# TencentCloudADP/youtu-rag

Hardware: AMD Instinct MI355X
Metric: retrieval QPS + recall@10 vs CPU ref, 10M×1024 corpus, 1/2/4/8 MI355X (higher is better)
Workload: dtype bf16

## Files before the change

youtu-rag_amd/csrc/hr_index.hip:

```cpp
#include "hr_internal.hpp"
#include "hr_kernels.hpp"

static thread_local std::string g_err;
int set_err(int code, const std::string& msg) {
    g_err = msg;
    return code;
}

static int async_drain(hr_index* h);

struct Persist {
    int mode = 1;
    bool ready = false;
    int64_t key_n = -1;
    const void* key_rows = nullptr;
    int key_S = 0, key_P = 0, key_ncu = 0;
    Scratch slot[kPersistSlots];
    DevBuf ar_qfrag, ar_mkeys, ar_floor, ar_pbuf, ar_pcnt, ar_dynq;
    int64_t st_qfrag = 0, st_mkeys = 0, st_floor = 0, st_pbuf = 0, st_pcnt = 0, st_dynq = 0;
    DevBuf ctl;
    uint32_t* host_err = nullptr;
    hipStream_t pst = nullptr;
    hipEvent_t posted[kPersistSlots] = {};
    hipEvent_t closed = nullptr;
// ... 429 lines not shown
    std::lock_guard<std::mutex> lk(h->mu);
    if (int rc = async_drain(h)) return rc;
    if (h->n + n > max_rows(h)) return set_err(HR_E_INVALID, "a shard holds at most 2^32 rows");
    if (n == 0) {
        if (first_row_out) *first_row_out = h->n;
        return HR_OK;
    }
    if (h->G > 1) return group_add_device(h, rows_dev, n, first_row_out, (hipStream_t)stream);
    if (int rc = set_device(h)) return rc;
    hipEvent_t ev;
    HIP_TRY(hipEventCreateWithFlags(&ev, hipEventDisableTiming));
    hipError_t e = hipEventRecord(ev, (hipStream_t)stream);
    if (e == hipSuccess) e = hipStreamWaitEvent(h->stream, ev, 0);
    (void)hipEventDestroy(ev);
    HIP_TRY(e);
    return add_impl<ADD_DEVICE>(h, rows_dev, 0, 0, n, first_row_out);
}

extern "C" int hr_index_remove(hr_index* h, const int64_t* rows, int64_t n) {
    if (!h || n < 0 || (n > 0 && !rows)) return set_err(HR_E_INVALID, "bad arguments");
    std::lock_guard<std::mutex> lk(h->mu);
    if (int rc = async_drain(h)) return rc;
    if (h->G > 1) return group_remove(h, rows, n);
    return index_remove_local(h, rows, n);
}

int index_remove_local(hr_index* h, const int64_t* rows, int64_t n) {
    if (int rc = set_device(h)) return rc;
    for (int64_t i = 0; i < n; ++i)
        if (rows[i] < 0 || rows[i] >= h->n) return set_err(HR_E_INVALID, "row out of range");
    int64_t lo = INT64_MAX, hi = -1;
    for (int64_t i = 0; i < n; ++i) {
        const int64_t r = rows[i];
        uint32_t& w = h->live_host[(size_t)(r >> 5)];
        const uint32_t bit = 1u << (r & 31);
        if (w & bit) {
            w &= ~bit;
            h->n_live--;
        }
        lo = std::min(lo, r >> 5);
        hi = std::max(hi, r >> 5);
    }
    if (hi >= 0) {
        HIP_TRY(hipMemcpyAsync(h->live + lo, h->live_host.data() + lo, (size_t)(hi - lo + 1) * 4,
                               hipMemcpyHostToDevice, h->stream));
        HIP_TRY(hipStreamSynchronize(h->stream));
    }
    return HR_OK;
}

extern "C" int hr_index_size(hr_index* h, int64_t* n_out, int64_t* n_live_out) {
    if (!h) return set_err(HR_E_INVALID, "null handle");
    std::lock_guard<std::mutex> lk(h->mu);
    if (n_out) *n_out = h->n;
    int64_t live = h->n_live;
    if (h->G > 1) {
        live = 0;
        for (hr_index* s : h->shards) live += s->n_live;
    }
    if (n_live_out) *n_live_out = live;
    return HR_OK;
}

extern "C" int hr_index_info(hr_index* h, int* dim_out, int* dtype_out, int* metric_out, int* n_dev_out) {
    if (!h) return set_err(HR_E_INVALID, "null handle");
    if (dim_out) *dim_out = h->dim;
    if (dtype_out) *dtype_out = h->dtype;
    if (metric_out) *metric_out = h->metric;
    if (n_dev_out) *n_dev_out = h->G;
    return HR_OK;
}

static int knob(const char* name, int dflt) {
    const char* v = getenv(name);
    return v && *v ? atoi(v) : dflt;
}
static const int kTailCus = knob("HIPRAG_TAIL_CUS", 32);
static const int kSampleMin = knob("HIPRAG_SAMPLE_MIN", 1024);
static const int kDynPct = knob("HIPRAG_DYN_PCT", 10);
static const int kRefreshEvery = std::max(0, knob("HIPRAG_REFRESH_EVERY", 0));
static int refresh_every(int64_t n_tiles) { return kRefreshEvery ? kRefreshEvery : (n_tiles <= 160 * 1024 ? 8 : 4); }
static const int kRefreshEvery8 = std::max(0, knob("HIPRAG_REFRESH_EVERY8", 0));
static int refresh_every8() { return kRefreshEvery8 ? kRefreshEvery8 : (kRefreshEvery ? kRefreshEvery : 16); }

struct Plan {
    int QB, Bp, P;
    int NG;
};

static int scan_lds_bytes(const hr_index* h, int QB) { return h->S * QB * 1024; }

static int make_plan(const hr_index* h, int B, Plan* p) {
    const int QB = (B > 32 && scan_lds_bytes(h, 2) <= 160 * 1024) ? 2 : 1;
    if (scan_lds_bytes(h, QB) > 160 * 1024)
        return set_err(HR_E_UNSUPPORTED, "dim too large for the LDS-resident query tile (max 2560)");
    p->QB = QB;
    constexpr int max_groups = 4;
    const int sdt = scan_dtype(h);
    p->NG = (QB == 2 && (sdt != F32 || wide_filter_ok(sdt, h->S))) ? std::max(1, std::min(max_groups, (B + 63) / 64)) : 1;
    if (QB == 1 && B > 32 && sdt != F32) p->NG = std::max(1, std::min(max_groups, (B + 31) / 32));
    if (p->NG > 1 && QB == 2 && wide_filter_ok(sdt, h->S)) p->NG = (p->NG + 1) & ~1;
    p->Bp = p->NG * QB * 32;
    const int pmax = sdt == F32 ? (QB == 2 ? 4 : 8) : 16;
    p->P = (h->S % 16 == 0 && pmax >= 16) ? 16 : (h->S % 8 == 0 && pmax >= 8 ? 8 : 4);
    return HR_OK;
}

static bool wide_plan(const hr_index* h, const Plan& pl, int np, bool tile_list) {
    const bool f32 = scan_dtype(h) == F32;
    const int max_parts = std::min(f32 ? 7 : 3, wide_max_parts(scan_dtype(h)));
    const bool parts_ok = np <= max_parts && (f32 || pl.NG == 2);
    return pl.NG >= 2 && pl.QB == 2 && !tile_list && (np == 1 || parts_ok) && wide_filter_ok(scan_dtype(h), h->S);
}

static void set_dyn_tail(ScanArgs& args, int64_t W, uint32_t* dyn_q) {
    const int pct = kDynPct;
    const int64_t per_wave = args.n_units / W;
    args.dyn_start = args.n_units;
    if (per_wave >= 8 && dyn_q) {
        const int64_t s_per = per_wave - std::max<int64_t>(2, per_wave * pct / 100);
        args.dyn_start = s_per * W;
        args.dyn_pct = pct;
        args.dyn_chunk = 2;
        args.dyn_q = dyn_q;
    }
}

template <int MT, int DT, int QB, int P, int MODE, bool NT, int TPB = kScanThreads, bool QM = false>
static int launch_scan_t(hr_index* h, Scratch& sc, int cus, const ScanArgs& a, hipStream_t st, int lds) {
    const int ng = std::max(1, a.ng);
    auto kern = scan_kernel<MT, DT, QB, P, MODE, NT, TPB, QM>();
    static std::mutex attr_mu;
    static int attr_lds[64] = {};
    static int occ[64][4] = {};
    const int dev = h->device & 63;
    const int bucket = lds <= 40 * 1024 ? 0 : lds <= 80 * 1024 ? 1 : lds <= 120 * 1024 ? 2 : 3;
    int per_cu;
    {
        std::lock_guard<std::mutex> lk(attr_mu);
        if (attr_lds[dev] < 160 * 1024) {
            HIP_TRY(hipFuncSetAttribute((const void*)kern, hipFuncAttributeMaxDynamicSharedMemorySize, 160 * 1024));
            attr_lds[dev] = 160 * 1024;
        }
        if (!occ[dev][bucket]) {
            int o = 0;
            HIP_TRY(hipOccupancyMaxActiveBlocksPerMultiprocessor(&o, kern, TPB, lds));
            occ[dev][bucket] = std::max(1, o);
        }
        per_cu = occ[dev][bucket];
    }
    int64_t blocks = std::max<int64_t>(1, std::min<int64_t>((int64_t)cus * per_cu / ng, (a.n_units + 7) / 8));
    if (ng > 1) blocks = std::max<int64_t>(8, blocks / 8 * 8);
    ScanArgs args = a;
    args.ng = ng;
    if (MODE == SCAN_FILTER) {
        const int64_t W = blocks * (TPB / 64);
        const int Bq = QB * 32;
        HIP_TRY(sc.pbuf.ensure((size_t)ng * Bq * W * kCapW * sizeof(float2)));
        HIP_TRY(sc.pcnt.ensure((size_t)ng * Bq * W * 4));
        HIP_TRY(sc.wtiles.ensure((size_t)ng * W * 4));
        args.wave_tiles = sc.wtiles.as<uint32_t>();
        sc.wtiles_valid = true;
        args.pbuf = sc.pbuf.as<float2>();
        args.pcnt = sc.pcnt.as<uint32_t>();
        args.capw = kCapW;
        sc.last_W = W;
        sc.last_Bp = Bq;
        sc.last_ng = ng;
        sc.last_capw = kCapW;
        h->last_scr = &sc;
        set_dyn_tail(args, W, sc.dyn_q.as<uint32_t>());
    }
    hipLaunchKernelGGL(kern, dim3((unsigned)(blocks * ng)), dim3(TPB), lds, st, args);
    HIP_TRY(hipGetLastError());
    return HR_OK;
}

template <int MT, int DT, int MODE>
static int launch_scan_p(hr_index* h, Scratch& sc, int cus, const Plan& pl, const ScanArgs& a, hipStream_t st,
                         bool qm = false) {
    int lds = scan_lds_bytes(h, pl.QB);
    if (MODE == SCAN_SAMPLE) lds = std::max(lds, (kScanThreads / 64) * pl.QB * 16 * 64 * 4 + 64);
    const bool dflt = pl.NG > 1 || MODE == SCAN_SAMPLE;
    if constexpr (MODE == SCAN_FILTER) {
        if (wide_plan(h, pl, a.np, a.tile_list != nullptr) && a.use_groups) {
            if (pl.NG == 4 && a.np == 1 && h->q256 && q256_filter_ok(scan_dtype(h), h->S)) {
                const int blocks = (int)std::max<int64_t>(1, std::min<int64_t>(cus, (a.n_units + 7) / 8));
                const int64_t W = (int64_t)blocks * 4;
                HIP_TRY(sc.pbuf.ensure((size_t)4 * 64 * W * kCapW * sizeof(float2)));
                HIP_TRY(sc.pcnt.ensure((size_t)4 * 64 * W * 4));
                sc.last_W = W;
                sc.last_Bp = 64;
                sc.last_ng = 4;
                sc.last_capw = kCapW;
                sc.wtiles_valid = false;
                h->last_scr = &sc;
                ScanArgs b = a;
                b.pbuf = sc.pbuf.as<float2>();
                b.pcnt = sc.pcnt.as<uint32_t>();
                b.capw = kCapW;
                if (int rc = launch_filter_q256(MT, DT, h->S, blocks, b, st)) return set_err(rc, "256-query FILTER launch failed");
                h->n_q256++;
                return HR_OK;
            }
            constexpr int wpb = 8;
            const int blocks = (int)std::max<int64_t>(1, std::min<int64_t>(cus, (a.n_units + wpb - 1) / wpb));
            const int64_t W = (int64_t)blocks * wpb;
            HIP_TRY(sc.pbuf.ensure((size_t)pl.NG * 64 * W * kCapW * sizeof(float2)));
            HIP_TRY(sc.pcnt.ensure((size_t)pl.NG * 64 * W * 4));
            sc.last_W = W;
            sc.last_Bp = 64;
            sc.last_ng = pl.NG;
            sc.last_capw = kCapW;
            sc.wtiles_valid = false;
            h->last_scr = &sc;
            for (int set = 0; set < pl.NG / 2; ++set) {
                ScanArgs b = a;
                b.qfrag = a.qfrag + (int64_t)set * 2 * h->S * 2 * 64 * 8;
                b.mkeys = a.mkeys + set * 128 * 32;
                b.floor_q = a.floor_q + set * 128;
                b.pbuf = sc.pbuf.as<float2>() + (int64_t)set * 2 * W * 64 * kCapW;
                b.pcnt = sc.pcnt.as<uint32_t>() + (int64_t)set * 2 * W * 64;
                b.capw = kCapW;
                if (int rc = launch_filter_wide(MT, DT, h->S, blocks, b, st)) return set_err(rc, "wide FILTER launch failed");
                h->n_wide++;
            }
            return HR_OK;
        }
    }
    if constexpr (MODE != SCAN_COLLECT) {
        if (qm) {
            if (pl.NG != 1 || !a.mask) return set_err(HR_E_INVALID, "per-query masks take one query group per pass");
            if (MODE == SCAN_FILTER) h->n_qmask++;
            constexpr bool QNT = MODE == SCAN_FILTER;
#define HR_SCAN_QM_CASE(QBv, Pv) \
    if (pl.QB == QBv && pl.P == Pv)  \
        return launch_scan_t<MT, DT, QBv, Pv, MODE, QNT, kScanThreads, true>(h, sc, cus, a, st, lds);
            if constexpr (DT == F32) {
                HR_SCAN_QM_CASE(1, 8) HR_SCAN_QM_CASE(1, 4) HR_SCAN_QM_CASE(2, 4)
            } else {
                HR_SCAN_QM_CASE(1, 16) HR_SCAN_QM_CASE(2, 16) HR_SCAN_QM_CASE(1, 8) HR_SCAN_QM_CASE(2, 8)
                HR_SCAN_QM_CASE(1, 4) HR_SCAN_QM_CASE(2, 4)
            }
#undef HR_SCAN_QM_CASE
            return set_err(HR_E_INVALID, "no per-query-mask scan variant for this plan");
        }
    }
#define HR_SCAN_CASE(QBv, Pv)                                                                     \
    if (pl.QB == QBv && pl.P == Pv)                                                               \
        return dflt ? launch_scan_t<MT, DT, QBv, Pv, MODE, false>(h, sc, cus, a, st, lds)         \
                    : launch_scan_t<MT, DT, QBv, Pv, MODE, true>(h, sc, cus, a, st, lds);
    if constexpr (DT == F32) {
        HR_SCAN_CASE(1, 8) HR_SCAN_CASE(1, 4) HR_SCAN_CASE(2, 4)
    } else {
        HR_SCAN_CASE(1, 16) HR_SCAN_CASE(2, 16) HR_SCAN_CASE(1, 8) HR_SCAN_CASE(2, 8) HR_SCAN_CASE(1, 4)
        HR_SCAN_CASE(2, 4)
    }
#undef HR_SCAN_CASE
    return set_err(HR_E_INVALID, "no scan variant for this plan");
}

static int launch_scan(hr_index* h, Scratch& sc, int cus, const Plan& pl, const ScanArgs& a, int mode,
                       hipStream_t st, bool qm = false) {
    return dispatch_dt(scan_dtype(h), [&](auto dt) -> int {
        constexpr int DT = decltype(dt)::value;
        auto go = [&](auto mt) -> int {
            constexpr int MT = decltype(mt)::value;
            if (mode == SCAN_SAMPLE) return launch_scan_p<MT, DT, SCAN_SAMPLE>(h, sc, cus, pl, a, st, qm);
            if (mode == SCAN_FILTER) return launch_scan_p<MT, DT, SCAN_FILTER>(h, sc, cus, pl, a, st, qm);
            return launch_scan_p<MT, DT, SCAN_COLLECT>(h, sc, cus, pl, a, st);
        };
        if constexpr (DT == F32) {
            if (mfma_type(h) == F16) return go(std::integral_constant<int, F16>{});
            return go(std::integral_constant<int, BF16>{});
        } else {
            return go(std::integral_constant<int, DT == F16 ? F16 : BF16>{});
        }
    });
}

template <int MODE>
static int launch_scan8(hr_index* h, Scratch& sc, int cus, const Plan& pl, const ScanArgs& a, hipStream_t st) {
    static_assert(MODE == SCAN_SAMPLE || MODE == SCAN_FILTER, "the collect pass reads the 16-bit rows");
    int lds = scan_lds_bytes(h, pl.QB);
    if (MODE == SCAN_SAMPLE) lds = std::max(lds, (kScanThreads / 64) * pl.QB * 16 * 64 * 4 + 64);
    const int S8 = h->S / 2;
    const int P8 = S8 % 16 == 0 ? 16 : (S8 % 8 == 0 ? 8 : (S8 % 4 == 0 ? 4 : 2));
    constexpr bool NT = MODE == SCAN_FILTER;
    if (MODE == SCAN_FILTER) h->n_shadow8++;
#define HR_SCAN8_CASE(QBv, Pv) \
    if (pl.QB == QBv && P8 == Pv) return launch_scan_t<F16, I8S, QBv, Pv, MODE, NT>(h, sc, cus, a, st, lds);
    HR_SCAN8_CASE(2, 16) HR_SCAN8_CASE(1, 16) HR_SCAN8_CASE(2, 8) HR_SCAN8_CASE(1, 8) HR_SCAN8_CASE(2, 4)
    HR_SCAN8_CASE(1, 4) HR_SCAN8_CASE(2, 2) HR_SCAN8_CASE(1, 2)
#undef HR_SCAN8_CASE
    return set_err(HR_E_INVALID, "no shadow-8 scan variant for this plan");
}

static int tail_cus(const hr_index* h) {
    return std::max(0, std::min(kTailCus, h->n_cu - 8));
}

static int persist_quiesce(hr_index* h) {
    Persist* ps = h->ps;
    if (!ps || !(ps->active || ps->launched)) return HR_OK;
    if (int rc = set_device(h)) return rc;
    PersistCtl* c = ps->ctl.as<PersistCtl>();
    if (ps->active)
        if (int rc = launch_persist_close(c, h->pre)) return rc;
    HIP_TRY(hipStreamSynchronize(h->pre));
    HIP_TRY(hipStreamSynchronize(ps->pst));
    HIP_TRY(hipMemsetAsync(&c->stop, 0, 4, ps->pst));
    HIP_TRY(hipStreamSynchronize(ps->pst));
    ps->active = ps->launched = false;
    if (ps->host_err && *(volatile uint32_t*)ps->host_err) {
        ps->timeouts++;
        ps->last_err = *(volatile uint32_t*)ps->host_err;
        *(volatile uint32_t*)ps->host_err = 0;
        HIP_TRY(hipMemset(&c->error, 0, 4));
    }
    return HR_OK;
}

static int persist_close(hr_index* h) {
    Persist* ps = h->ps;
    if (!ps || !ps->active) return HR_OK;
    if (int rc = set_device(h)) return rc;
    if (int rc = launch_persist_close(ps->ctl.as<PersistCtl>(), h->pre)) return rc;
    HIP_TRY(hipEventRecord(ps->closed, h->pre));
    HIP_TRY(hipStreamWaitEvent(ps->pst, ps->closed, 0));
    HIP_TRY(hipMemsetAsync(&ps->ctl.as<PersistCtl>()->stop, 0, 4, ps->pst));
    ps->active = false;
    return HR_OK;
}

static void persist_free(hr_index* h) {
    Persist* ps = h->ps;
    if (!ps) return;
    (void)persist_quiesce(h);
    ps->drop_views();
    for (auto& sc : ps->slot) sc.release_all();
    for (DevBuf* b : {&ps->ar_qfrag, &ps->ar_mkeys, &ps->ar_floor, &ps->ar_pbuf, &ps->ar_pcnt, &ps->ar_dynq, &ps->ctl})
        b->release();
    for (auto& e : ps->posted)
        if (e) (void)hipEventDestroy(e);
    if (ps->closed) (void)hipEventDestroy(ps->closed);
    if (ps->pst) (void)hipStreamDestroy(ps->pst);
    if (ps->host_err) (void)hipHostFree(ps->host_err);
    delete ps;
    h->ps = nullptr;
}

static bool persist_wanted(hr_index* h, const Plan& pl, int np, bool early, const uint64_t* mask_dev, int64_t n_tiles) {
    const int mode = h->ps ? h->ps->mode : 1;
    if (mode == 0 || !early || mask_dev || np != 1 || pl.NG != 1 || pl.QB != 2 || h->stripe_G != 1) return false;
    if (!(scan_dtype(h) != F32 ? pl.P == 16 : pl.P == 4)) return false;
    return mode == 2 || (n_tiles >= 128 * 1024 && n_tiles <= 160 * 1024);
}

static int persist_configure(hr_index* h, const Plan& pl) {
    if (!h->ps) h->ps = new Persist();
    Persist& ps = *h->ps;
    const int64_t n_tiles = (h->n + 31) / 32;
    const int nwg = h->n_cu - tail_cus(h);
    if (ps.ready && ps.key_n == h->n && ps.key_rows == h->rows && ps.key_S == h->S && ps.key_P == pl.P &&
        ps.key_ncu == h->n_cu)
        return HR_OK;
    if (int rc = persist_quiesce(h)) return rc;
    if ((n_tiles + 7) / 8 < nwg) return set_err(HR_E_UNSUPPORTED, "shard too small for the persistent FILTER");
    if (!ps.pst) {
        HIP_TRY(index_stream_create(h, &ps.pst, true));
        for (auto& e : ps.posted) HIP_TRY(hipEventCreateWithFlags(&e, hipEventDisableTiming));
        HIP_TRY(hipEventCreateWithFlags(&ps.closed, hipEventDisableTiming));
        HIP_TRY(hipHostMalloc((void**)&ps.host_err, 64));
        *ps.host_err = 0;
// ... 2073 lines not shown
```

youtu-rag_amd/csrc/hr_kernels.hpp:

```cpp
#pragma once
#include "hr_common.hpp"

namespace hr {

template <int DT, bool SYNTH>
__global__ __launch_bounds__(256) void k_store(const float* __restrict__ in, uint64_t seed, int64_t gen_base, int64_t n,
                                               int dim, int S, int metric, int64_t lrow0, uint8_t* __restrict__ rows,
                                               unsigned long long* max_norm2_bits,
                                               const int64_t* __restrict__ dest = nullptr, int sG = 1, int ss = 0) {
    const int lane = threadIdx.x & 63;
    const int64_t r = (int64_t)blockIdx.x * 4 + (threadIdx.x >> 6);
    if (r >= n) return;
    const int64_t grow = SYNTH ? gen_base + stripe_row(lrow0 + r, sG, ss) : 0;
    auto src = [&](int d) -> float {
        if (d >= dim) return 0.0f;
        return SYNTH ? gen_elem(seed, grow, dim, d) : in[r * dim + d];
    };
    double inv = 1.0;
    bool scale = false;
    if (metric == COSINE) {
        double p = 0.0;
        for (int d = lane; d < dim; d += 64) {
            double x = (double)src(d);
            p = p + x * x;
// ... 116 lines not shown
    }
    double e1 = 0.0, nh = 0.0, qn = 0.0;
    const int qg = (b >> 5) / QB, qb = (b >> 5) % QB;
    auto put = [&](int d, float x) {
        const float y = scale ? (float)((double)x * inv) : x;
        q32[(int64_t)b * dpad + d] = y;
        const uint16_t h = quant_mt<MT>(y);
        const float dq = dequant_mt<MT>(h);
        const int s = d >> 4, sl = (b & 31) + 32 * ((d >> 3) & 1), jj = d & 7;
        qfrag[((((int64_t)qg * S + s) * QB + qb) * 64 + sl) * 8 + jj] = h;
        const double e = (double)y - (double)dq;
        e1 += e * e;
        nh += (double)dq * (double)dq;
        qn = qn + (double)y * (double)y;
    };
#pragma unroll
    for (int j = 0; j < kPrepJ; ++j)
        if (lane + 64 * j < dpad) put(lane + 64 * j, v[j]);
    for (int d = lane + 64 * kPrepJ; d < dpad; d += 64) put(d, src(d));
    e1 = wave_butterfly_sum(e1);
    nh = wave_butterfly_sum(nh);
    qn = wave_butterfly_sum(qn);
    if (lane == 0) {
        qerr[4 * b] = __builtin_sqrt(e1);
        qerr[4 * b + 1] = __builtin_sqrt(nh);
        qerr[4 * b + 2] = qn;
        qerr[4 * b + 3] = 0.0;
    }
}

constexpr int vmcnt_only(int n) { return 0x0F70 | (n & 15) | (((n >> 4) & 3) << 14); }

__device__ inline void stage_lds(u32x4* dst, const u32x4* src, int n) {
    constexpr int U = 8;
    const int st = blockDim.x;
    int i = threadIdx.x;
    for (; i + (U - 1) * st < n; i += U * st) {
        u32x4 v[U];
#pragma unroll
        for (int j = 0; j < U; ++j) v[j] = src[i + j * st];
#pragma unroll
        for (int j = 0; j < U; ++j) dst[i + j * st] = v[j];
    }
    for (; i < n; i += st) dst[i] = src[i];
}

struct ScanArgs {
    const uint8_t* rows;
    const uint32_t* live;
    const uint32_t* mask;
    const uint16_t* qfrag;
    int S;
    int64_t n_units;
    int64_t sample_stride;
    const uint32_t* tile_list;
    uint32_t* mkeys;
    int np;
    int64_t part_tiles;
    int64_t pstride;
    const float* floor_q;
    int use_groups;
    uint32_t* cnt;
    float2* buf;
    int cap;
    int refresh_every;
    int publish;
    int private_bufs;
    int wave_major;
    int strided;
    float2* pbuf;
    uint32_t* pcnt;
    int capw;
    int64_t dyn_start;
    int dyn_chunk;
    uint32_t* dyn_q;
    const float* xnorm;
    uint32_t* wave_tiles;
    int ng;
    int early_refresh;
    int teams;
    int dyn_pct;
    int stagger;
    const float* rscale;
};


constexpr int kPersistSlots = 3;
constexpr int kPersistRing = 4096;
struct PersistCtl {
    uint32_t gate;
    uint32_t posted;
    uint32_t next_epoch;
    uint32_t stop;
    uint32_t error;
    uint32_t runs;
    uint32_t opened;
    uint32_t pad;
    uint32_t slot_fail[4];
    unsigned long long arr[kPersistRing];
    unsigned long long t_end[kPersistRing];
    unsigned long long t_post[kPersistRing], t_start0[kPersistRing], t_start1[kPersistRing], t_end0[kPersistRing];
};
struct PersistLaunch {
    ScanArgs a;
    int64_t st_qfrag, st_mkeys, st_floor, st_pbuf, st_pcnt, st_dynq;
    PersistCtl* ctl;
    uint32_t* host_err;
    uint32_t e0;
    uint32_t idle_ticks;
};

template <int MT>
__device__ inline f32x16 mfma32(const u32x4& a, const u32x4& b, const f32x16& c) {
    if constexpr (MT == BF16)
        return __builtin_amdgcn_mfma_f32_32x32x16_bf16(__builtin_bit_cast(bf16x8, a), __builtin_bit_cast(bf16x8, b), c,
                                                        0, 0, 0);
    else
        return __builtin_amdgcn_mfma_f32_32x32x16_f16(__builtin_bit_cast(f16x8, a), __builtin_bit_cast(f16x8, b), c, 0,
                                                       0, 0);
}

template <int MT, int DT, bool NT = true>
struct XFrag;
#ifndef HR_CORPUS_NT
#define HR_CORPUS_NT 1
#endif
#ifndef HR_DIAG
#define HR_DIAG 0
#endif
#ifndef HR_ROTATE_ROUNDS
#define HR_ROTATE_ROUNDS 1
#endif
__device__ inline int64_t wave_uniform(int64_t v) {
    const uint32_t lo = (uint32_t)__builtin_amdgcn_readfirstlane((int)(uint32_t)v);
    const uint32_t hi = (uint32_t)__builtin_amdgcn_readfirstlane((int)(uint32_t)((uint64_t)v >> 32));
    return (int64_t)(((uint64_t)hi << 32) | lo);
}
__device__ inline uint32_t scalar_word(const uint32_t* p, int64_t i) {
    return ((const __attribute__((address_space(4))) uint32_t*)p)[i];
}
template <bool NT>
__device__ inline u32x4 corpus_load(const uint8_t* p) {
#if HR_CORPUS_NT
    if constexpr (NT) return __builtin_nontemporal_load((const u32x4*)p);
#endif
    return *(const u32x4*)p;
}
template <int MT, bool NT>
struct XFrag<MT, BF16, NT> {
    static constexpr int kLoads = 1;
    static constexpr int kSteps = 1;
    u32x4 v;
    __device__ inline void load(const uint8_t* rows, int64_t c, int lane) {
        v = corpus_load<NT>(rows + c * 1024 + lane * 16);
    }
    __device__ inline u32x4 get(int = 0) const { return v; }
};
template <int MT, bool NT>
struct XFrag<MT, F16, NT> {
    static constexpr int kLoads = 1;
    static constexpr int kSteps = 1;
    u32x4 v;
    __device__ inline void load(const uint8_t* rows, int64_t c, int lane) {
        v = corpus_load<NT>(rows + c * 1024 + lane * 16);
    }
    __device__ inline u32x4 get(int = 0) const { return v; }
};
template <int MT, bool NT>
struct XFrag<MT, F32, NT> {
    static constexpr int kLoads = 2;
    static constexpr int kSteps = 1;
    u32x4 a, b;
    __device__ inline void load(const uint8_t* rows, int64_t c, int lane) {
        a = corpus_load<NT>(rows + c * 2048 + lane * 16);
        b = corpus_load<NT>(rows + c * 2048 + 1024 + lane * 16);
    }
    __device__ inline u32x4 get(int = 0) const {
        typedef float f32x4 __attribute__((ext_vector_type(4)));
        typedef float f32x8 __attribute__((ext_vector_type(8)));
        const f32x4 fa = __builtin_bit_cast(f32x4, a);
        const f32x4 fb = __builtin_bit_cast(f32x4, b);
        const f32x8 f = __builtin_shufflevector(fa, fb, 0, 1, 2, 3, 4, 5, 6, 7);
        if constexpr (MT == BF16) {
            return __builtin_bit_cast(u32x4, __builtin_convertvector(f, bf16x8));
        } else {
            return __builtin_bit_cast(u32x4, __builtin_convertvector(f, f16x8));
        }
    }
};

template <bool NT>
struct XFrag<F16, I8S, NT> {
    static constexpr int kLoads = 1;
    static constexpr int kSteps = 2;
    u32x4 v;
    __device__ inline void load(const uint8_t* rows, int64_t c, int lane) {
        v = corpus_load<NT>(rows + c * 1024 + lane * 16);
    }
    __device__ inline u32x4 get(int ks) const {
        typedef _Float16 f16x2 __attribute__((ext_vector_type(2)));
        const uint32_t w0 = ks ? v[2] : v[0], w1 = ks ? v[3] : v[1];
        const f16x2 off = {(_Float16)1152.0f, (_Float16)1152.0f};
        auto cv = [&](uint32_t w, uint32_t sel) -> uint32_t {
            const uint32_t m = __builtin_amdgcn_perm(0x64646464u, w, sel);
            return __builtin_bit_cast(uint32_t, __builtin_bit_cast(f16x2, m) - off);
        };
        u32x4 o;
        o[0] = cv(w0, 0x04010400u);
        o[1] = cv(w0, 0x04030402u);
        o[2] = cv(w1, 0x04010400u);
        o[3] = cv(w1, 0x04030402u);
        return o;
    }
};

__device__ inline int acc_query(int qb, int i, int half) { return qb * 32 + (i & 3) + 8 * (i >> 2) + 4 * half; }

template <int CTRL>
__device__ __forceinline__ uint32_t dpp_u32(uint32_t v) {
    return (uint32_t)__builtin_amdgcn_update_dpp((int)v, (int)v, CTRL, 0xF, 0xF, false);
}
__device__ __forceinline__ float half_min32(float f) {
    f = fminf(f, __builtin_bit_cast(float, dpp_u32<0xB1>(__builtin_bit_cast(uint32_t, f))));
    f = fminf(f, __builtin_bit_cast(float, dpp_u32<0x4E>(__builtin_bit_cast(uint32_t, f))));
    f = fminf(f, __builtin_bit_cast(float, dpp_u32<0x141>(__builtin_bit_cast(uint32_t, f))));
    f = fminf(f, __builtin_bit_cast(float, dpp_u32<0x140>(__builtin_bit_cast(uint32_t, f))));
    return fminf(f, __builtin_bit_cast(float, __builtin_amdgcn_ds_swizzle(__builtin_bit_cast(int, f), 0x401F)));
}
__device__ __forceinline__ uint32_t wave_or(uint32_t x) {
    x |= dpp_u32<0xB1>(x);
    x |= dpp_u32<0x4E>(x);
    x |= dpp_u32<0x141>(x);
    x |= dpp_u32<0x140>(x);
    return (uint32_t)(__builtin_amdgcn_readlane((int)x, 0) | __builtin_amdgcn_readlane((int)x, 16) |
                      __builtin_amdgcn_readlane((int)x, 32) | __builtin_amdgcn_readlane((int)x, 48));
}
__device__ __forceinline__ float half_kth_largest(float f, int j) {
    const int lane = __lane_id();
    for (int r = 0; r < 32 - j; ++r) {
        const float m = half_min32(f);
        const uint64_t b = __ballot(f == m);
        const uint32_t bh = lane >= 32 ? (uint32_t)(b >> 32) : (uint32_t)b;
        if ((lane & 31) == __builtin_ctz(bh)) f = __builtin_inff();
    }
    return half_min32(f);
}

enum { SCAN_SAMPLE = 0, SCAN_FILTER = 1, SCAN_COLLECT = 2 };

template <int MT, int DT, int QB, int P, int MODE, bool NT, int TPB, bool LEAN = false, bool QM = false>
__device__ __forceinline__ void scan_body(ScanArgs a) {
    constexpr bool FILTER = MODE != SCAN_SAMPLE;
    constexpr bool priv = MODE == SCAN_FILTER;
    static_assert(!LEAN || MODE == SCAN_FILTER, "the lean body is a FILTER");
    static_assert(!QM || (!LEAN && MODE != SCAN_COLLECT && DT != I8S), "per-query masks: the plain SAMPLE / FILTER");
    if constexpr (LEAN) {
        a.ng = 1;
        a.np = 1;
        a.part_tiles = (int64_t)1 << 62;
        a.mask = nullptr;
        a.tile_list = nullptr;
        a.strided = 1;
        a.wave_major = 1;
        a.teams = 0;
        a.use_groups = 1;
        a.publish = 1;
    }
    extern __shared__ __attribute__((aligned(16))) uint8_t lds[];
    int tid_ = threadIdx.x;
    if constexpr (LEAN) asm volatile("" : "+v"(tid_));
    const int tid = tid_;
    const int lane = tid & 63;
    const int half = lane >> 5;
    const int g = lane & 31;

    const int ng = a.ng;
    const int bx = blockIdx.x;
    const int grp = ng > 1 ? (bx >> 3) % ng : 0;
    const int64_t nrb = gridDim.x / ng;
    const int64_t rb = ng > 1 ? (int64_t)((bx >> 3) / ng) * 8 + (bx & 7) : bx;
    {
        constexpr int Bq = QB * 32;
        a.qfrag += (int64_t)grp * a.S * QB * 64 * 8;
        a.mkeys += grp * Bq * 32;
        a.floor_q += grp * Bq;
        if (a.cnt) a.cnt += grp * Bq;
        if (a.buf) a.buf += (int64_t)grp * Bq * a.cap;
        if (a.dyn_q) a.dyn_q += grp * 16;
    }
    const int64_t Wg = nrb * (blockDim.x >> 6);
    const int64_t w = rb * (blockDim.x >> 6) + (tid >> 6);
    const int64_t wg = (int64_t)grp * Wg + w;
    const int64_t wrg = a.wave_major ? (int64_t)(tid >> 6) * nrb + rb : w;
    const bool teams = MODE == SCAN_FILTER && a.np > 1 && a.teams && a.strided;
    const int tp = teams ? (int)(wrg % a.np) : 0;
    const int64_t W = teams ? (Wg - tp + a.np - 1) / a.np : Wg;
    const int64_t wr = teams ? wrg / a.np : wrg;
    const int64_t t_off = teams ? (int64_t)tp * a.part_tiles : 0;
    const int64_t n_units = teams ? std::max<int64_t>(0, std::min<int64_t>(a.n_units - t_off, a.part_tiles)) : a.n_units;
    int64_t dyn_start = a.dyn_start;
    if (teams) {
        const int64_t per_wave = n_units / W;
        dyn_start = n_units;
        if (a.dyn_start < a.n_units && per_wave >= 8)
            dyn_start = (per_wave - std::max<int64_t>(2, per_wave * a.dyn_pct / 100)) * W;
    }
    uint32_t* const dyn_ctr = a.dyn_q ? a.dyn_q + tp : nullptr;
    const bool dyn = MODE == SCAN_FILTER && dyn_start < n_units;
    const int64_t n_static = dyn ? dyn_start : n_units;
    const int64_t base = n_static / W, rem = n_static % W;
    const bool strided = a.strided != 0 && (a.np == 1 || teams);
    const int64_t u0 = strided ? 0 : wr * base + (wr < rem ? wr : rem);
    const int64_t u1 = strided ? (wr < n_static ? (n_static - 1 - wr) / W + 1 : 0) : u0 + base + (wr < rem ? 1 : 0);
    const int64_t stride = FILTER ? 1 : a.sample_stride;
    constexpr int KS = XFrag<MT, DT, NT>::kSteps;
    const int S = a.S / KS;
    __builtin_assume(S >= P);
    bool in_static = true;
    const int64_t full_rounds = n_static / W;
    auto tile_at = [&](int64_t u) -> int64_t {
        if (strided && in_static) {
            int64_t pos = wr;
            if (HR_ROTATE_ROUNDS && u < full_rounds) {
                const uint32_t rot = (uint32_t)((uint64_t)u * 2654435761ull) % (uint32_t)W;
                pos += rot;
                if (pos >= W) pos -= W;
            }
            u = u * W + pos;
        }
        const int64_t i = wave_uniform(t_off + u * stride);
        return a.tile_list ? (int64_t)scalar_word(a.tile_list, i) : i;
    };

    const int n_q16 = a.S * QB * 64;
    if constexpr (!LEAN) {
        if (!(HR_DIAG & 8)) {
            const __amdgpu_buffer_rsrc_t qr =
                __builtin_amdgcn_make_buffer_rsrc((void*)a.qfrag, (short)0, n_q16 * 16, 0x00020000);
            const int wv = __builtin_amdgcn_readfirstlane(tid >> 6);
            for (int c = wv * 64; c < n_q16; c += (int)blockDim.x)
                __builtin_amdgcn_raw_ptr_buffer_load_lds(qr, (__attribute__((address_space(3))) void*)(lds + c * 16), 16,
                                                         lane * 16, c * 16, 0, 0);
        }
    }
    XFrag<MT, DT, NT> ring[P];
    const bool ring0 = u0 < u1;
    if (ring0) {
        const int64_t c0 = tile_at(u0) * S;
#pragma unroll
        for (int i = 0; i < P; ++i) ring[i].load(a.rows, c0 + i, lane);
    }
    if constexpr (LEAN) {
        stage_lds((u32x4*)lds, (const u32x4*)a.qfrag, n_q16);
    } else {
        if (ring0) __builtin_amdgcn_s_waitcnt(vmcnt_only(P * XFrag<MT, DT, NT>::kLoads));
        else __builtin_amdgcn_s_waitcnt(vmcnt_only(0));
    }
    __syncthreads();

    if (u0 >= u1 && FILTER) {
        if (priv && lane < QB * 32) {
            if constexpr (LEAN)
                __hip_atomic_store(&a.pcnt[wg * (QB * 32) + lane], 0u, __ATOMIC_RELAXED, __HIP_MEMORY_SCOPE_AGENT);
            else
                a.pcnt[wg * (QB * 32) + lane] = 0;
        }
        if (a.wave_tiles && lane == 0) a.wave_tiles[wg] = 0u;
        return;
    }
    uint32_t mycnt = 0;
    float2* const wave_buf = priv ? a.pbuf + wg * (QB * 32) * a.capw : nullptr;

    const u32x4* qs = (const u32x4*)lds;

    float th[QB][16], gmax[QB][16];
    int64_t part = (u0 < u1 ? tile_at(u0) : 0) / a.part_tiles;
    int64_t part_end = (part + 1) * a.part_tiles;
    uint32_t* gkq[QB];
#pragma unroll
    for (int qb = 0; qb < QB; ++qb) gkq[qb] = a.mkeys + part * a.pstride + (qb * 32 + 4 * half) * 32 + g;
#pragma unroll
    for (int qb = 0; qb < QB; ++qb)
#pragma unroll
        for (int i = 0; i < 16; ++i) {
            gmax[qb][i] = -__builtin_inff();
            th[qb][i] = -__builtin_inff();
        }

    auto refresh_load = [&](uint32_t (&key)[QB][16]) {
#pragma unroll
        for (int qb = 0; qb < QB; ++qb)
#pragma unroll
            for (int i = 0; i < 16; ++i)
                key[qb][i] = __hip_atomic_load(gkq[qb] + 32 * ((i & 3) + 8 * (i >> 2)), __ATOMIC_RELAXED,
                                               __HIP_MEMORY_SCOPE_AGENT);
    };
    auto refresh_apply = [&](uint32_t (&key)[QB][16], bool publish, bool floor) {
#pragma unroll
        for (int qb = 0; qb < QB; ++qb)
#pragma unroll
            for (int i = 0; i < 16; ++i) {
                key[qb][i] = key[qb][i] > HR_KEY_NEG_INF ? key[qb][i] : HR_KEY_NEG_INF;
                if (publish && a.publish && gmax[qb][i] > key2f(key[qb][i])) {
                    atomicMax(gkq[qb] + 32 * ((i & 3) + 8 * (i >> 2)), f2key(gmax[qb][i]));
                    key[qb][i] = f2key(gmax[qb][i]);
                }
            }
        for (int p = 0; p < a.np; ++p) {
            if (p == part) continue;
            const int64_t off = (p - part) * a.pstride;
            uint32_t k2[QB][16];
#pragma unroll
            for (int qb = 0; qb < QB; ++qb)
#pragma unroll
                for (int i = 0; i < 16; ++i)
                    k2[qb][i] = __hip_atomic_load(gkq[qb] + off + 32 * ((i & 3) + 8 * (i >> 2)), __ATOMIC_RELAXED,
                                                  __HIP_MEMORY_SCOPE_AGENT);
#pragma unroll
            for (int qb = 0; qb < QB; ++qb)
#pragma unroll
                for (int i = 0; i < 16; ++i) {
                    const uint32_t v = k2[qb][i] > HR_KEY_NEG_INF ? k2[qb][i] : HR_KEY_NEG_INF;
                    key[qb][i] = key[qb][i] < v ? key[qb][i] : v;
                }
        }
#pragma unroll
        for (int qb = 0; qb < QB; ++qb)
#pragma unroll
            for (int i = 0; i < 16; ++i) {
                float f = key2f(key[qb][i]);
#pragma unroll
                for (int off = 16; off >= 1; off >>= 1) f = fminf(f, __shfl_xor(f, off, 64));
                gmax[qb][i] = -__builtin_inff();
                if (floor) f = fmaxf(f, a.floor_q[acc_query(qb, i, half)]);
                th[qb][i] = fmaxf(th[qb][i], f);
            }
    };
    auto refresh = [&](bool publish) {
        if (!a.use_groups) {
#pragma unroll
            for (int qb = 0; qb < QB; ++qb)
#pragma unroll
                for (int i = 0; i < 16; ++i) {
                    gmax[qb][i] = -__builtin_inff();
                    th[qb][i] = fmaxf(th[qb][i], a.floor_q[acc_query(qb, i, half)]);
                }
            return;
        }
        uint32_t key[QB][16];
        refresh_load(key);
        refresh_apply(key, publish, true);
    };
    auto flush = [&]() {
#pragma unroll
        for (int qb = 0; qb < QB; ++qb)
#pragma unroll
            for (int i = 0; i < 16; ++i) {
                if (gmax[qb][i] > -__builtin_inff())
                    atomicMax(gkq[qb] + 32 * ((i & 3) + 8 * (i >> 2)), f2key(gmax[qb][i]));
                gmax[qb][i] = -__builtin_inff();
            }
    };
    if (FILTER) refresh(false);


    auto grab_issue = [&]() -> uint32_t {
        uint32_t v = 0;
        if (lane == 0) v = atomicAdd(dyn_ctr, 1u);
        return v;
    };
    auto grab_resolve = [&](uint32_t v) -> int64_t {
        v = (uint32_t)__builtin_amdgcn_readfirstlane((int)v);
        const int64_t u = dyn_start + (int64_t)v * a.dyn_chunk;
        return u < n_units ? u : -1;
    };
    uint32_t rkey[QB][16];
    const bool early_refresh = !LEAN && DT != I8S && !QM && a.early_refresh != 0;
    int64_t u = u0, u_end = u1, pend = -1, done = 0;
    const int roff = a.stagger ? __builtin_amdgcn_readfirstlane((tid >> 6) % a.refresh_every) : 0;
    uint32_t graw = 0;
    bool issued = false;
    if (dyn && u0 >= u1) {
        in_static = false;
        u = grab_resolve(grab_issue());
        if (u < 0) u = u_end = 0;
        else u_end = std::min<int64_t>(u + a.dyn_chunk, n_units);
    }
    while (u < u_end) {
        if (dyn && !issued && u + 2 >= u_end) {
            graw = grab_issue();
            issued = true;
        }
        if (dyn && u + 1 == u_end) pend = grab_resolve(graw);
        const int64_t t = wave_uniform(tile_at(u));
        int64_t tn = t;
        if (u + 1 < u_end) {
            tn = tile_at(u + 1);
        } else if (pend >= 0) {
            const bool st = in_static;
            in_static = false;
            tn = tile_at(pend);
            in_static = st;
        }
        tn = wave_uniform(tn);
        if (t >= part_end) {
            if (MODE != SCAN_COLLECT && a.use_groups) flush();
            const int64_t np_ = t / a.part_tiles;
#pragma unroll
            for (int qb = 0; qb < QB; ++qb) gkq[qb] += (np_ - part) * a.pstride;
            part = np_;
            part_end = (part + 1) * a.part_tiles;
        }
        const bool rdue = MODE == SCAN_FILTER && a.use_groups && early_refresh && !(HR_DIAG & 2) &&
                          ((done + 1 + roff) % a.refresh_every) == 0;
        if (rdue) {
            refresh_load(rkey);
            asm volatile("" ::: "memory");
        }
        f32x16 acc[QB];
#pragma unroll
        for (int qb = 0; qb < QB; ++qb)
#pragma unroll
            for (int i = 0; i < 16; ++i) acc[qb][i] = 0.0f;
        const int rg = slot_row(t, g);

        uint32_t allow = QM ? 0u : scalar_word(a.live, t);
        if (!QM && a.mask) allow &= scalar_word(a.mask, t);
        uint32_t aw = 0;
        if constexpr (QM) {
            aw = a.mask[t * 64 + lane];
            asm volatile("" ::: "memory");
        }
        float rsc = 1.0f;
        if constexpr (DT == I8S) {
            rsc = a.rscale[t * 32 + rg];
            asm volatile("" ::: "memory");
        }
        for (int sb = 0; sb < S; sb += P) {
            const bool same = sb + P < S;
            const int64_t nc = same ? t * S + sb + P : tn * S;
#pragma unroll
            for (int i = 0; i < P; ++i) {
                u32x4 xf[KS];
#pragma unroll
                for (int ks = 0; ks < KS; ++ks) xf[ks] = ring[i].get(ks);
                ring[i].load(a.rows, nc + i, lane);
#pragma unroll
// ... 23 lines not shown
                in_static = false;
                u = pend;
                u_end = std::min<int64_t>(u + a.dyn_chunk, n_units);
                pend = -1;
                issued = false;
            } else {
                break;
            }
            continue;
        }
        if (a.xnorm) {
            const float xs = a.xnorm[t * 32 + rg];
            const float xmul = 2.0f;
#pragma unroll
            for (int qb = 0; qb < QB; ++qb)
#pragma unroll
                for (int i = 0; i < 16; ++i) acc[qb][i] = __builtin_fmaf(xmul, acc[qb][i], -xs);
        }
        if constexpr (DT == I8S) {
#pragma unroll
            for (int qb = 0; qb < QB; ++qb)
#pragma unroll
                for (int i = 0; i < 16; ++i) acc[qb][i] *= rsc;
        }
        const bool ok = (allow >> rg) & 1u;
#define HR_OKR(qb, i) (QM ? ((aw >> ((qb) * 16 + (i))) & 1u) != 0 : ok)
        const uint32_t row = (uint32_t)(t * 32 + rg);
        uint32_t regs = 0;
#pragma unroll
        for (int qb = 0; qb < QB; ++qb)
#pragma unroll
            for (int i = 0; i < 16; ++i) {
                const float v = HR_OKR(qb, i) ? acc[qb][i] : -__builtin_inff();
                gmax[qb][i] = fmaxf(gmax[qb][i], v);
                if (FILTER) regs |= (__ballot(HR_OKR(qb, i) && v >= th[qb][i]) != 0 ? 1u : 0u) << (qb * 16 + i);
            }
        if (FILTER && regs && !(HR_DIAG & 1)) {
#pragma unroll
            for (int qb = 0; qb < QB; ++qb)
#pragma unroll
                for (int i = 0; i < 16; ++i) {
                    if (!((regs >> (qb * 16 + i)) & 1u)) continue;
                    const float v = acc[qb][i];
                    const bool pass = HR_OKR(qb, i) && v >= th[qb][i];
                    const uint64_t m = __ballot(pass);
                    if (m) {
#pragma unroll
                        for (int h = 0; h < 2; ++h) {
                            const uint32_t mh = (uint32_t)(m >> (32 * h));
                            if (priv && mh) {
                                const int q = acc_query(qb, i, h);
                                const uint32_t basepos = (uint32_t)__builtin_amdgcn_readlane((int)mycnt, q);
                                if (pass && half == h) {
                                    const uint32_t pos = basepos + __builtin_popcount(mh & ((1u << g) - 1u));
                                    if (pos < (uint32_t)a.capw) {
                                        if constexpr (LEAN)
                                            __hip_atomic_store((uint64_t*)&wave_buf[q * a.capw + pos],
                                                               ((uint64_t)row << 32) | __builtin_bit_cast(uint32_t, v),
                                                               __ATOMIC_RELAXED, __HIP_MEMORY_SCOPE_AGENT);
                                        else
                                            wave_buf[q * a.capw + pos] = make_float2(v, __builtin_bit_cast(float, row));
                                    }
                                }
                                mycnt += (lane == q) ? (uint32_t)__builtin_popcount(mh) : 0u;
                            } else if (!priv && mh) {
                                const int q = acc_query(qb, i, h);
                                const int leader = 32 * h + __builtin_ctz(mh);
                                uint32_t basepos = 0;
                                if (lane == leader) basepos = atomicAdd(&a.cnt[q], (uint32_t)__builtin_popcount(mh));
                                basepos = __shfl(basepos, leader, 64);
                                if (pass && half == h) {
                                    const uint32_t pos = basepos + __builtin_popcount(mh & ((1u << g) - 1u));
                                    if (pos < (uint32_t)a.cap)
                                        a.buf[(int64_t)q * a.cap + pos] = make_float2(v, __builtin_bit_cast(float, row));
                                }
                            }
                        }
                    }
                }
        }
#undef HR_OKR
        ++done;
        if (MODE == SCAN_FILTER && !(HR_DIAG & 2) && ((done + roff) % a.refresh_every) == 0) {
            if (rdue) refresh_apply(rkey, true, false);
            else refresh(true);
        }
        if (u + 1 < u_end) {
            ++u;
        } else if (pend >= 0 && done < n_units) {
            in_static = false;
            u = pend;
            u_end = std::min<int64_t>(u + a.dyn_chunk, n_units);
            pend = -1;
            issued = false;
        } else {
            break;
        }
    }

    if (priv && lane < QB * 32) {
        if constexpr (LEAN)
            __hip_atomic_store(&a.pcnt[wg * (QB * 32) + lane], mycnt, __ATOMIC_RELAXED, __HIP_MEMORY_SCOPE_AGENT);
        else
            a.pcnt[wg * (QB * 32) + lane] = mycnt;
    }
    if (a.wave_tiles && lane == 0) a.wave_tiles[wg] = (uint32_t)done;
    if (!FILTER && a.publish) {
        constexpr int NE = QB * 16 * 64;
        float* red = (float*)lds;
        int64_t* partw = (int64_t*)(red + 8 * NE);
        const int wv = tid >> 6;
        __syncthreads();
#pragma unroll
        for (int qb = 0; qb < QB; ++qb)
#pragma unroll
            for (int i = 0; i < 16; ++i) red[wv * NE + (qb * 16 + i) * 64 + lane] = gmax[qb][i];
        if (lane == 0) partw[wv] = u0 < u1 ? part : -1;
        __syncthreads();
        int64_t p0 = -1;
        bool same = true;
        const int nw = blockDim.x >> 6;
        for (int v = 0; v < nw; ++v) {
            if (partw[v] < 0) continue;
            if (p0 < 0) p0 = partw[v];
            same = same && partw[v] == p0;
        }
        if (!same) {
            flush();
        } else if (p0 >= 0) {
            for (int e = tid; e < NE; e += blockDim.x) {
                float m = -__builtin_inff();
                for (int v = 0; v < nw; ++v) m = fmaxf(m, red[v * NE + e]);
                if (m > -__builtin_inff()) {
                    const int l = e & 63, ri = (e >> 6) & 15, qb = e >> 10;
                    const int q = qb * 32 + 4 * (l >> 5) + (ri & 3) + 8 * (ri >> 2);
                    atomicMax(a.mkeys + p0 * a.pstride + q * 32 + (l & 31), f2key(m));
                }
            }
        }
    }
}


template <int MT, int DT, int QB, int P, bool NT, int TPB, bool QM = false>
__global__ __launch_bounds__(TPB, TPB >= 512 ? 2 : 1) void k_scan_sample(ScanArgs a) {
    scan_body<MT, DT, QB, P, SCAN_SAMPLE, NT, TPB, false, QM>(a);
}
template <int MT, int DT, int QB, int P, bool NT, int TPB, bool QM = false>
__global__ __launch_bounds__(TPB, TPB >= 512 ? 2 : 1) void k_scan_filter(ScanArgs a) {
    scan_body<MT, DT, QB, P, SCAN_FILTER, NT, TPB, false, QM>(a);
}
template <int MT, int DT, int QB, int P, bool NT, int TPB>
__global__ __launch_bounds__(TPB, TPB >= 512 ? 2 : 1) void k_scan_collect(ScanArgs a) {
    scan_body<MT, DT, QB, P, SCAN_COLLECT, NT, TPB>(a);
}
template <int MT, int DT, int QB, int P, int MODE, bool NT, int TPB, bool QM = false>
constexpr auto scan_kernel() {
    if constexpr (MODE == SCAN_SAMPLE) return &k_scan_sample<MT, DT, QB, P, NT, TPB, QM>;
    else if constexpr (MODE == SCAN_FILTER) return &k_scan_filter<MT, DT, QB, P, NT, TPB, QM>;
    else return &k_scan_collect<MT, DT, QB, P, NT, TPB>;
}

template <int MT, int DT, int QB>
__global__ __launch_bounds__(256) void k_debug_approx(const uint8_t* __restrict__ rows, const uint16_t* __restrict__ qfrag,
                                                      int S, int64_t n_tiles, const float* __restrict__ xnorm,
                                                      float* __restrict__ out,
                                                      const float* __restrict__ rscale = nullptr) {
    extern __shared__ __attribute__((aligned(16))) uint8_t lds[];
    stage_lds((u32x4*)lds, (const u32x4*)qfrag, S * QB * 64);
    __syncthreads();
    const int lane = threadIdx.x & 63;
    const int64_t t = (int64_t)blockIdx.x * 4 + (threadIdx.x >> 6);
    if (t >= n_tiles) return;
    const u32x4* qs = (const u32x4*)lds;
    f32x16 acc[QB];
#pragma unroll
    for (int qb = 0; qb < QB; ++qb)
#pragma unroll
        for (int i = 0; i < 16; ++i) acc[qb][i] = 0.0f;
    constexpr int KS = XFrag<MT, DT>::kSteps;
    for (int s = 0; s < S / KS; ++s) {
        XFrag<MT, DT> x;
        x.load(rows, t * (S / KS) + s, lane);
#pragma unroll
        for (int ks = 0; ks < KS; ++ks) {
            const u32x4 xf = x.get(ks);
#pragma unroll
            for (int qb = 0; qb < QB; ++qb)
                acc[qb] = mfma32<MT>(qs[((s * KS + ks) * QB + qb) * 64 + lane], xf, acc[qb]);
        }
    }
    const int64_t ncol = n_tiles * 32;
    const int rg = slot_row(t, lane & 31);
    if (rscale) {
        const float rsc = rscale[t * 32 + rg];
#pragma unroll
        for (int qb = 0; qb < QB; ++qb)
#pragma unroll
            for (int i = 0; i < 16; ++i) acc[qb][i] *= rsc;
    }
    const float xs = xnorm ? xnorm[t * 32 + rg] : 0.0f;
#pragma unroll
    for (int qb = 0; qb < QB; ++qb)
#pragma unroll
        for (int i = 0; i < 16; ++i)
            out[(int64_t)acc_query(qb, i, lane >> 5) * ncol + t * 32 + rg] =
                xnorm ? __builtin_fmaf(2.0f, acc[qb][i], -xs) : acc[qb][i];
}

__device__ inline void block_bitonic_desc(uint64_t* s, int n) {
    for (int k = 2; k <= n; k <<= 1) {
        for (int j = k >> 1; j > 0; j >>= 1) {
            for (int i = threadIdx.x; i < n; i += blockDim.x) {
                int ixj = i ^ j;
                if (ixj > i) {
                    uint64_t x = s[i], y = s[ixj];
                    bool desc = (i & k) == 0;
                    if (desc ? (x < y) : (x > y)) {
                        s[i] = y;
                        s[ixj] = x;
                    }
                }
            }
            __syncthreads();
        }
    }
}

static __global__ __attribute__((unused)) __launch_bounds__(256) void k_floor_kth(const uint32_t* __restrict__ mkeys,
                                                                                   float* __restrict__ floor_q, int B,
                                                                                   int kj) {
    const int q = blockIdx.x * 4 + (threadIdx.x >> 6);
    if (q >= B) return;
    const uint32_t k = mkeys[(int64_t)q * 32 + (threadIdx.x & 31)];
    const float t = half_kth_largest(key2f(k > HR_KEY_NEG_INF ? k : HR_KEY_NEG_INF), kj);
    if ((threadIdx.x & 63) == 0) floor_q[q] = fmaxf(floor_q[q], t);
}

static __global__ __attribute__((unused)) __launch_bounds__(64) void k_floor_kth_parts(const uint32_t* __restrict__ mkeys,
                                                                                        float* __restrict__ floor_q,
                                                                                        int Bp, int np, int kj) {
// ... 286 lines not shown
```

Before: 31520.

## Share threshold refresh across waves via an LDS row in shadow-8 filter scan

```diff
diff --git a/youtu-rag_amd/csrc/hr_index.hip b/youtu-rag_amd/csrc/hr_index.hip
--- a/youtu-rag_amd/csrc/hr_index.hip
+++ b/youtu-rag_amd/csrc/hr_index.hip
@@ -535,6 +535,7 @@
 static int refresh_every(int64_t n_tiles) { return kRefreshEvery ? kRefreshEvery : (n_tiles <= 160 * 1024 ? 8 : 4); }
 static const int kRefreshEvery8 = std::max(0, knob("HIPRAG_REFRESH_EVERY8", 0));
 static int refresh_every8() { return kRefreshEvery8 ? kRefreshEvery8 : (kRefreshEvery ? kRefreshEvery : 16); }
+static const int kRefreshLds = knob("HIPRAG_REFRESH_LDS", 1);
 
 struct Plan {
     int QB, Bp, P;
@@ -579,10 +580,10 @@
     }
 }
 
-template <int MT, int DT, int QB, int P, int MODE, bool NT, int TPB = kScanThreads, bool QM = false>
+template <int MT, int DT, int QB, int P, int MODE, bool NT, int TPB = kScanThreads, bool QM = false, bool THL = false>
 static int launch_scan_t(hr_index* h, Scratch& sc, int cus, const ScanArgs& a, hipStream_t st, int lds) {
     const int ng = std::max(1, a.ng);
-    auto kern = scan_kernel<MT, DT, QB, P, MODE, NT, TPB, QM>();
+    auto kern = scan_kernel<MT, DT, QB, P, MODE, NT, TPB, QM, THL>();
     static std::mutex attr_mu;
     static int attr_lds[64] = {};
     static int occ[64][4] = {};
@@ -733,7 +734,7 @@
 }
 
 template <int MODE>
-static int launch_scan8(hr_index* h, Scratch& sc, int cus, const Plan& pl, const ScanArgs& a, hipStream_t st) {
+static int launch_scan8(hr_index* h, Scratch& sc, int cus, const Plan& pl, const ScanArgs& a_, hipStream_t st) {
     static_assert(MODE == SCAN_SAMPLE || MODE == SCAN_FILTER, "the collect pass reads the 16-bit rows");
     int lds = scan_lds_bytes(h, pl.QB);
     if (MODE == SCAN_SAMPLE) lds = std::max(lds, (kScanThreads / 64) * pl.QB * 16 * 64 * 4 + 64);
@@ -741,8 +742,19 @@
     const int P8 = S8 % 16 == 0 ? 16 : (S8 % 8 == 0 ? 8 : (S8 % 4 == 0 ? 4 : 2));
     constexpr bool NT = MODE == SCAN_FILTER;
     if (MODE == SCAN_FILTER) h->n_shadow8++;
-#define HR_SCAN8_CASE(QBv, Pv) \
-    if (pl.QB == QBv && P8 == Pv) return launch_scan_t<F16, I8S, QBv, Pv, MODE, NT>(h, sc, cus, a, st, lds);
+    ScanArgs a = a_;
+    a.th_off = 0;
+    if (MODE == SCAN_FILTER && kRefreshLds && a.use_groups && a.np <= 5 && lds + pl.QB * 32 * 4 <= 160 * 1024) {
+        a.th_off = lds;
+        lds += pl.QB * 32 * 4;
+    }
+#define HR_SCAN8_CASE(QBv, Pv)                                                                                      \
+    if (pl.QB == QBv && P8 == Pv) {                                                                                 \
+        if constexpr (MODE == SCAN_FILTER)                                                                          \
+            if (a.th_off)                                                                                           \
+                return launch_scan_t<F16, I8S, QBv, Pv, MODE, NT, kScanThreads, false, true>(h, sc, cus, a, st, lds); \
+        return launch_scan_t<F16, I8S, QBv, Pv, MODE, NT>(h, sc, cus, a, st, lds);                                  \
+    }
     HR_SCAN8_CASE(2, 16) HR_SCAN8_CASE(1, 16) HR_SCAN8_CASE(2, 8) HR_SCAN8_CASE(1, 8) HR_SCAN8_CASE(2, 4)
     HR_SCAN8_CASE(1, 4) HR_SCAN8_CASE(2, 2) HR_SCAN8_CASE(1, 2)
 #undef HR_SCAN8_CASE
diff --git a/youtu-rag_amd/csrc/hr_kernels.hpp b/youtu-rag_amd/csrc/hr_kernels.hpp
--- a/youtu-rag_amd/csrc/hr_kernels.hpp
+++ b/youtu-rag_amd/csrc/hr_kernels.hpp
@@ -222,6 +222,7 @@
     int dyn_pct;
     int stagger;
     const float* rscale;
+    int th_off;
 };
 
 
@@ -388,8 +389,9 @@
 
 enum { SCAN_SAMPLE = 0, SCAN_FILTER = 1, SCAN_COLLECT = 2 };
 
-template <int MT, int DT, int QB, int P, int MODE, bool NT, int TPB, bool LEAN = false, bool QM = false>
+template <int MT, int DT, int QB, int P, int MODE, bool NT, int TPB, bool LEAN = false, bool QM = false, bool THL = false>
 __device__ __forceinline__ void scan_body(ScanArgs a) {
+    static_assert(!THL || (DT == I8S && !LEAN && !QM && MODE == SCAN_FILTER), "the shared refresh: the shadow-8 FILTER");
     constexpr bool FILTER = MODE != SCAN_SAMPLE;
     constexpr bool priv = MODE == SCAN_FILTER;
     static_assert(!LEAN || MODE == SCAN_FILTER, "the lean body is a FILTER");
@@ -496,6 +498,11 @@
         if (ring0) __builtin_amdgcn_s_waitcnt(vmcnt_only(P * XFrag<MT, DT, NT>::kLoads));
         else __builtin_amdgcn_s_waitcnt(vmcnt_only(0));
     }
+    constexpr bool TH_ROW = THL;
+    float* const th_row = (float*)(lds + (TH_ROW ? a.th_off : 0));
+    if constexpr (TH_ROW) {
+        if (tid < QB * 32) th_row[tid] = -__builtin_inff();
+    }
     __syncthreads();
 
     if (u0 >= u1 && FILTER) {
@@ -603,6 +610,63 @@
     };
     if (FILTER) refresh(false);
 
+    constexpr int SW = 2 * QB;
+    constexpr int NSL = QB * 32 / (2 * SW);
+    constexpr int kThParts = 5;
+    int th_r = tid >> 6;
+    [[maybe_unused]] auto slice_apply = [&]() {
+        const int s = __builtin_amdgcn_readfirstlane(th_r % NSL);
+        ++th_r;
+        int ln = lane;
+        asm volatile("" : "+v"(ln));
+        const __amdgpu_buffer_rsrc_t kr =
+            __builtin_amdgcn_make_buffer_rsrc((void*)a.mkeys, (short)0, (int)(a.np * a.pstride * 4), 0x00020000);
+        uint32_t sl[kThParts][SW];
+#pragma unroll
+        for (int p = 0; p < kThParts; ++p) {
+            const int pp = p < a.np ? p : a.np - 1;
+            const int soff = (int)(pp * a.pstride + s * (64 * SW)) * 4;
+            if constexpr (SW == 4) {
+                const u32x4 v = __builtin_amdgcn_raw_buffer_load_b128(kr, ln * 16, soff, 16);
+                sl[p][0] = v.x, sl[p][1] = v.y, sl[p][2] = v.z, sl[p][3] = v.w;
+            } else if constexpr (SW == 2) {
+                const auto v = __builtin_amdgcn_raw_buffer_load_b64(kr, ln * 8, soff, 16);
+                sl[p][0] = v[0], sl[p][1] = v[1];
+            } else {
+                sl[p][0] = __builtin_amdgcn_raw_buffer_load_b32(kr, ln * 4, soff, 16);
+            }
+        }
+        if (a.publish) {
+#pragma unroll
+            for (int qb = 0; qb < QB; ++qb)
+#pragma unroll
+                for (int i = 0; i < 16; ++i)
+                    if (gmax[qb][i] > th[qb][i])
+                        atomicMax(gkq[qb] + 32 * ((i & 3) + 8 * (i >> 2)), f2key(gmax[qb][i]));
+        }
+        uint32_t m = sl[0][0];
+#pragma unroll
+        for (int p = 0; p < kThParts; ++p)
+#pragma unroll
+            for (int j = 0; j < SW; ++j) m = m < sl[p][j] ? m : sl[p][j];
+        float f = key2f(m > HR_KEY_NEG_INF ? m : HR_KEY_NEG_INF);
+#pragma unroll
+        for (int off = 32 / SW / 2; off >= 1; off >>= 1) f = fminf(f, __shfl_xor(f, off, 64));
+        if ((ln & (32 / SW - 1)) == 0) th_row[s * (2 * SW) + ln / (32 / SW)] = f;
+        asm volatile("" ::: "memory");
+#pragma unroll
+        for (int qb = 0; qb < QB; ++qb)
+#pragma unroll
+            for (int j = 0; j < 4; ++j) {
+                typedef float f32x4 __attribute__((ext_vector_type(4)));
+                const f32x4 r = *(const f32x4*)(th_row + qb * 32 + 8 * j + 4 * (ln >> 5));
+#pragma unroll
+                for (int c = 0; c < 4; ++c) {
+                    th[qb][4 * j + c] = fmaxf(th[qb][4 * j + c], r[c]);
+                    gmax[qb][4 * j + c] = -__builtin_inff();
+                }
+            }
+    };
 
     auto grab_issue = [&]() -> uint32_t {
         uint32_t v = 0;
@@ -792,7 +856,8 @@
 #undef HR_OKR
         ++done;
         if (MODE == SCAN_FILTER && !(HR_DIAG & 2) && ((done + roff) % a.refresh_every) == 0) {
-            if (rdue) refresh_apply(rkey, true, false);
+            if constexpr (TH_ROW) slice_apply();
+            else if (rdue) refresh_apply(rkey, true, false);
             else refresh(true);
         }
         if (u + 1 < u_end) {
@@ -860,13 +925,20 @@
 __global__ __launch_bounds__(TPB, TPB >= 512 ? 2 : 1) void k_scan_filter(ScanArgs a) {
     scan_body<MT, DT, QB, P, SCAN_FILTER, NT, TPB, false, QM>(a);
 }
+namespace lds_refresh {
+template <int MT, int DT, int QB, int P, bool NT, int TPB>
+__global__ __launch_bounds__(TPB, TPB >= 512 ? 2 : 1) void k_scan_filter(ScanArgs a) {
+    scan_body<MT, DT, QB, P, SCAN_FILTER, NT, TPB, false, false, true>(a);
+}
+}
 template <int MT, int DT, int QB, int P, bool NT, int TPB>
 __global__ __launch_bounds__(TPB, TPB >= 512 ? 2 : 1) void k_scan_collect(ScanArgs a) {
     scan_body<MT, DT, QB, P, SCAN_COLLECT, NT, TPB>(a);
 }
-template <int MT, int DT, int QB, int P, int MODE, bool NT, int TPB, bool QM = false>
+template <int MT, int DT, int QB, int P, int MODE, bool NT, int TPB, bool QM = false, bool THL = false>
 constexpr auto scan_kernel() {
     if constexpr (MODE == SCAN_SAMPLE) return &k_scan_sample<MT, DT, QB, P, NT, TPB, QM>;
+    else if constexpr (MODE == SCAN_FILTER && THL) return &lds_refresh::k_scan_filter<MT, DT, QB, P, NT, TPB>;
     else if constexpr (MODE == SCAN_FILTER) return &k_scan_filter<MT, DT, QB, P, NT, TPB, QM>;
     else return &k_scan_collect<MT, DT, QB, P, NT, TPB>;
 }
```

New measurement: 32410, median of 6. 1.03x the previous value.
